# at-cg/PHI

Measured on AMD Instinct MI355X. Metric: read Gbases/s scored (49-hap MHC graph stand-in synMHC-49); reads resident in HBM, parsing and H2D excluded, higher is better.
Workload: dtype u64

## Files before the change

phi_amd/csrc/dp_events.hip:

```cpp
#include <hip/hip_runtime.h>
#include "phi_kernels.h"
#include "dp_dev.h"

#define CHK PHI_DP_CHUNK
#define RING PHI_DP_RING
enum { DP_SEQ = 0, DP_ROW = 1, DP_PATH = 2 };

__global__ void __launch_bounds__(256) phi_event_flags_kernel(const int32_t *__restrict__ walk_vtx, int64_t n_entries,
                                                              const int32_t *__restrict__ cvtx, uint8_t *__restrict__ flags)
{
    for (int64_t e = (int64_t)blockIdx.x * blockDim.x + threadIdx.x; e < n_entries; e += (int64_t)gridDim.x * blockDim.x)
        flags[e] = cvtx[walk_vtx[e]] >= 0;
}

__global__ void phi_event_off_kernel(const phi_ent_t *__restrict__ ev_e, int64_t n_ev, const int64_t *__restrict__ walk_off,
                                     int32_t n_walks, int64_t *__restrict__ ev_off)
{
    const int h = blockIdx.x * blockDim.x + threadIdx.x;
    if (h > n_walks) return;
    const int64_t key = walk_off[h];
    int64_t lo = 0, hi = n_ev;
    while (lo < hi) {
        const int64_t mid = (lo + hi) >> 1;
        if ((int64_t)ev_e[mid] < key) lo = mid + 1; else hi = mid;
    }
    ev_off[h] = lo;
}

void phi_launch_event_flags(hipStream_t st, const int32_t *walk_vtx, int64_t n_entries, const int32_t *cvtx, uint8_t *flags)
{
    if (n_entries <= 0) return;
    int64_t nb = (n_entries + 255) / 256;
    if (nb > 4096) nb = 4096;
    hipLaunchKernelGGL(phi_event_flags_kernel, dim3((unsigned)nb), dim3(256), 0, st, walk_vtx, n_entries, cvtx, flags);
}

void phi_launch_event_off(hipStream_t st, const phi_ent_t *ev_e, int64_t n_ev, const int64_t *walk_off, int32_t n_walks,
                          int64_t *ev_off)
{
    hipLaunchKernelGGL(phi_event_off_kernel, dim3((unsigned)((n_walks + 1 + 63) / 64)), dim3(64), 0, st, ev_e, n_ev,
                       walk_off, n_walks, ev_off);
}

#define EVF_STAGE 3072
__global__ void __launch_bounds__(256) phi_dp_event_fill_kernel(const phi_ent_t *__restrict__ ev_e, int64_t n_ev,
                                                                const int32_t *__restrict__ walk_vtx,
                                                                const int32_t *__restrict__ cvtx,
                                                                const int64_t *__restrict__ walk_off, int32_t n_walks,
                                                                const uint8_t *__restrict__ e_out,
                                                                const int64_t *__restrict__ g_off,
                                                                const uint8_t *__restrict__ g_span,
                                                                const uint8_t *__restrict__ a_weight,
                                                                const phi_ent_t *__restrict__ a_e1,
                                                                const int32_t *__restrict__ wpre, int64_t n_entries,
                                                                uint4 *__restrict__ ev)
{
    __shared__ uint32_t s_e1[EVF_STAGE];
    __shared__ uint8_t s_sw[EVF_STAGE];
    __shared__ int64_t s_rng[2];
    const int64_t n_blocks = (n_ev + 255) / 256;
    for (int64_t blk = blockIdx.x; blk < n_blocks; blk += gridDim.x) {
        const int64_t i = blk * 256 + threadIdx.x;
        const bool in = i < n_ev;
        const int64_t e = ev_e[in ? i : n_ev - 1];
        const int64_t e1st = ((int64_t)__builtin_amdgcn_readfirstlane((int)(e >> 32)) << 32) | (uint32_t)__builtin_amdgcn_readfirstlane((int)(uint32_t)e);
        int lo = phi_walk_of_entry(walk_off, n_walks, e1st);
        if (__ballot(e >= walk_off[lo + 1]) != 0ull) lo = phi_walk_of_entry(walk_off, n_walks, e, lo);
        const int64_t eb = walk_off[lo];
        const int64_t x0 = e - 29 > eb ? e - 29 : eb;
        const int64_t xe = e + 31 < n_entries ? e + 31 : n_entries;
        const int64_t g_lo = g_off[x0], g_e = g_off[e], g_hi = g_off[e + 1], g_fe = g_off[xe];
        if (threadIdx.x == 0) s_rng[0] = g_lo;
        if (i == (n_ev < blk * 256 + 256 ? n_ev : blk * 256 + 256) - 1) s_rng[1] = g_fe;
        __syncthreads();
        const int64_t gb = s_rng[0], ge = s_rng[1];
        const bool staged = ge - gb <= EVF_STAGE;
        if (staged)
            for (int64_t j = threadIdx.x; j < ge - gb; j += 256) {
                s_e1[j] = a_e1[gb + j];
                s_sw[j] = (uint8_t)(g_span[gb + j] | (a_weight[gb + j] ? 0x80 : 0));
            }
        __syncthreads();
        if (in) {
            unsigned long long w[4] = {0, 0, 0, 0};
            int total = 0;
            int32_t sb_extra = 0;
            auto count = [&](int a) {
                if (a > 30) return;
                total++;
                const unsigned long long one = 1ull << (8 * (a & 7));
                if ((a >> 3) == 0) w[0] += one; else if ((a >> 3) == 1) w[1] += one; else if ((a >> 3) == 2) w[2] += one; else w[3] += one;
            };
            const uint32_t e32 = (uint32_t)e;
            if (staged) {
                for (int64_t g = g_lo - gb; g < g_hi - gb; g++) {
                    const uint32_t sw = s_sw[g];
                    if (sw & 0x80) count((int)(e32 - (s_e1[g] - (sw & 0x7F))));
                }
                for (int64_t g = g_e - gb; g < g_fe - gb; g++) {
                    const uint32_t sw = s_sw[g];
                    sb_extra += (sw & 0x80) && (int64_t)s_e1[g] - (int64_t)(sw & 0x7F) < e;
                }
            } else {
                for (int64_t g = g_lo; g < g_hi; g++)
                    if (a_weight[g]) count((int)(e - ((int64_t)a_e1[g] - g_span[g])));
                for (int64_t g = g_e; g < g_fe; g++) sb_extra += a_weight[g] && (int64_t)a_e1[g] - g_span[g] < e;
            }
            const bool ovf = total > 255;
            unsigned long long carry = 0;
#pragma unroll
            for (int q = 0; q < 4; q++) {
                w[q] = w[q] * 0x0101010101010101ull + carry * 0x0101010101010101ull;
                carry = w[q] >> 56;
            }
            w[3] = (w[3] & 0x00FFFFFFFFFFFFFFull) | ((unsigned long long)e_out[e] << 56);
            const int32_t base = wpre[g_off[eb]];
            uint4 A;
            A.x = (uint32_t)cvtx[walk_vtx[e]] | (ovf ? 0x80000000u : 0u);
            A.y = (uint32_t)e;
            A.z = (uint32_t)(wpre[g_hi] - base);
            A.w = (uint32_t)(wpre[g_e] - base + sb_extra);
            ev[i * 3 + 0] = A;
            ev[i * 3 + 1] = make_uint4((uint32_t)w[0], (uint32_t)(w[0] >> 32), (uint32_t)w[1], (uint32_t)(w[1] >> 32));
            ev[i * 3 + 2] = make_uint4((uint32_t)w[2], (uint32_t)(w[2] >> 32), (uint32_t)w[3], (uint32_t)(w[3] >> 32));
        }
        __syncthreads();
    }
}

void phi_launch_dp_event_fill(hipStream_t st, const PhiDpEventArgs &A, const uint8_t *e_out, const int32_t *walk_vtx,
                              const int32_t *cvtx, const phi_ent_t *a_e1, const int32_t *wpre, int64_t n_entries)
{
    if (A.n_ev <= 0) return;
    int64_t nb = (A.n_ev + 255) / 256;
    if (nb > 16384) nb = 16384;
    hipLaunchKernelGGL(phi_dp_event_fill_kernel, dim3((unsigned)nb), dim3(256), 0, st, A.ev_e, A.n_ev, walk_vtx, cvtx,
                       A.walk_off, A.n_walks, e_out, A.g_off, A.g_span, A.a_weight, a_e1, wpre, n_entries,
                       reinterpret_cast<uint4 *>(A.ev));
}

__device__ __forceinline__ unsigned long long ev_key(int32_t val, int lane)
{
    return ((unsigned long long)(uint32_t)(val - NEG) << 8) | (unsigned long long)(255 - lane);
}
__device__ __forceinline__ unsigned long long ev_max_u53(unsigned long long a, unsigned long long b)
{
    double r;
    asm("v_max_f64 %0, %1, %2" : "=v"(r) : "v"(__longlong_as_double((long long)a)), "v"(__longlong_as_double((long long)b)));
    return (unsigned long long)__double_as_longlong(r);
}
#define EV_DPP64(x, ctrl, rm, bc)                                                                                             \
    (((unsigned long long)(uint32_t)__builtin_amdgcn_update_dpp((int)((x) >> 32), (int)((x) >> 32), ctrl, rm, 0xF, bc) << 32) | \
     (uint32_t)__builtin_amdgcn_update_dpp((int)(uint32_t)(x), (int)(uint32_t)(x), ctrl, rm, 0xF, bc))
__device__ __forceinline__ void ev_wave_max2_key(unsigned long long a, unsigned long long b, unsigned long long &ma, unsigned long long &mb)
{
    a = ev_max_u53(a, EV_DPP64(a, 0x121, 0xF, false)); b = ev_max_u53(b, EV_DPP64(b, 0x121, 0xF, false));
    a = ev_max_u53(a, EV_DPP64(a, 0x122, 0xF, false)); b = ev_max_u53(b, EV_DPP64(b, 0x122, 0xF, false));
    a = ev_max_u53(a, EV_DPP64(a, 0x124, 0xF, false)); b = ev_max_u53(b, EV_DPP64(b, 0x124, 0xF, false));
    a = ev_max_u53(a, EV_DPP64(a, 0x128, 0xF, false)); b = ev_max_u53(b, EV_DPP64(b, 0x128, 0xF, false));
    a = ev_max_u53(a, EV_DPP64(a, 0x142, 0xA, false)); b = ev_max_u53(b, EV_DPP64(b, 0x142, 0xA, false));
    a = ev_max_u53(a, EV_DPP64(a, 0x143, 0xC, false)); b = ev_max_u53(b, EV_DPP64(b, 0x143, 0xC, false));
    ma = ((unsigned long long)(uint32_t)__builtin_amdgcn_readlane((int)(a >> 32), 63) << 32) | (uint32_t)__builtin_amdgcn_readlane((int)(uint32_t)a, 63);
    mb = ((unsigned long long)(uint32_t)__builtin_amdgcn_readlane((int)(b >> 32), 63) << 32) | (uint32_t)__builtin_amdgcn_readlane((int)(uint32_t)b, 63);
}

__device__ int32_t ev_count_inside(const PhiDpEventArgs &A, int64_t es, int64_t e)
{
    int32_t n = 0;
    for (int64_t x = es; x <= e; x++)
        for (int64_t g = A.g_off[x]; g < A.g_off[x + 1]; g++)
            if (A.a_weight[g] && x - A.g_span[g] >= es) n++;
    return n;
}

template <int NW, int MODE>
__global__ void __launch_bounds__(NW * 64) phi_dp_events_kernel(PhiDpEventArgs A)
{
    static_assert(NW == 2 || NW == 4, "65..128 or 129..256 walks");
    constexpr int NT = NW * 64;
    constexpr int D = NW == 2 ? 8 : 4;
    constexpr int P = D / 2;
    constexpr int QD = NW == 2 ? 32 : 16;
    constexpr int RNG = NW == 2 ? RING : 512;
    __shared__ int4 s_rec[2][CHK][2];
    __shared__ int4 s_top[RNG];
    __shared__ uint4 s_ev[D][3][NT];
    __shared__ int32_t s_qs[QD][NT], s_qE[QD][NT], s_qK[QD][NT];
    const int32_t q_limit = A.q_limit > 0 && A.q_limit < QD ? A.q_limit : (QD == 32 ? 32 : QD);
    __shared__ unsigned long long s_red[NW];
    __shared__ int32_t s_oidx[NT];

    const int h = threadIdx.x;
    const bool has_walk = h < A.n_walks;
    const int64_t eb = has_walk ? A.walk_off[h] : 0;
    const int64_t ee = has_walk ? A.walk_off[h + 1] : 0;
    const int32_t sb = MODE == DP_PATH ? (int32_t)blockIdx.x : 0;
    const int32_t kbeg = MODE == DP_PATH ? A.blk_lo[sb] : 0, kend = MODE == DP_PATH ? A.blk_lo[sb + 1] : A.n_k;
    const int64_t vb = !has_walk ? 0 : MODE == DP_PATH ? (int64_t)A.blk_ev[(int64_t)sb * A.lane_stride + h] : A.ev_off[h];
    const int64_t ve = has_walk ? A.ev_off[h + 1] : 0;
    int64_t vi = vb;
    int64_t wl = vb;
    const uint4 *evg = reinterpret_cast<const uint4 *>(A.ev);

    uint4 wtmp[P][3];
    int64_t whi = vb;
    auto issue = [&]() {
        whi = min(ve, vi + D);
#pragma unroll
        for (int j = 0; j < P; j++) {
            const int64_t x = (ve > vb) ? min(wl + j, ve - 1) : 0;
            wtmp[j][0] = evg[x * 3 + 0]; wtmp[j][1] = evg[x * 3 + 1]; wtmp[j][2] = evg[x * 3 + 2];
        }
    };
    auto land = [&]() {
#pragma unroll
        for (int j = 0; j < P; j++) {
            const int64_t x = wl + j;
            if (x < whi) {
                const int sl = (int)(x & (D - 1));
                s_ev[sl][0][h] = wtmp[j][0]; s_ev[sl][1][h] = wtmp[j][1]; s_ev[sl][2][h] = wtmp[j][2];
            }
        }
        wl = max(wl, min(whi, wl + P));
    };
    if (A.n_ev > 0) { issue(); land(); issue(); land(); }
    uint4 cA = make_uint4(0xFFFFFFFFu, 0, 0, 0);
    if (vi < ve) cA = s_ev[vi & (D - 1)][0][h];

    int32_t qh = 0, qt = 0;
    int32_t M = NEGK, sL = 0, Emax = NEG;
    if (MODE == DP_PATH) { sL = -1; if (has_walk) M = A.blk_S[(int64_t)sb * A.lane_stride + h]; }

    const int32_t n_steps = kend - kbeg;
    const int n_chunks = (n_steps + CHK - 1) / CHK;
    auto stage = [&](int c) {
        const int b = c & 1;
        const int32_t s0 = kbeg + c * CHK;
        const int32_t ns = min(CHK, kend - s0);
        const int4 *src = reinterpret_cast<const int4 *>(A.k_rec + (int64_t)s0 * 8);
        int4 *dst = &s_rec[b][0][0];
        for (int i = h; i < ns * 2; i += NT) dst[i] = src[i];
    };
    stage(0);
    __syncthreads();

    for (int c = 0; c < n_chunks; c++) {
        const int b = c & 1;
        if (c + 1 < n_chunks) stage(c + 1);
        const int32_t s0 = kbeg + c * CHK;
        const int32_t ns = min(CHK, kend - s0);
        int4 ra = s_rec[b][0][0], rb = s_rec[b][0][1];
        for (int i = 0; i < ns; i++) {
            const int inx = min(i + 1, CHK - 1);
            const int4 na = s_rec[b][inx][0], nb = s_rec[b][inx][1];
            if ((c | i) && (i & (P - 1)) == 0) issue();
            if ((c | i) && (i & (P - 1)) == P / 2) {
                land();
                if (vi < ve) cA = s_ev[vi & (D - 1)][0][h];
            }
            const int32_t k = s0 + i;
            const int32_t flags = ra.x;
            const bool active = (int32_t)(cA.x & 0x7FFFFFFFu) == k;

            int32_t E = NEG, Eh = -1, Esrc = -1;
            if (flags & PHI_DP_NEED_ENTRY) {
                dp_eval_entry<RNG, true>(ra, rb, k, s_top, A.k_in_packed, reinterpret_cast<const int4 *>(A.tops), A.cost, E, Eh, Esrc);
                if (h == 0) { A.ent_src[k] = Esrc; A.ent_h[k] = Eh; }
            }

            int32_t dmax = NEG;
            int32_t oidx = 255;
            if (active) {
                const int64_t e = (int64_t)cA.y;
                const bool ovf = (cA.x >> 31) != 0;
                const int32_t t = (int32_t)(e - eb);
                const int32_t End = (int32_t)cA.z, SB = (int32_t)cA.w;
                const int sl = (int)(vi & (D - 1));
                const uint8_t *gb = reinterpret_cast<const uint8_t *>(&s_ev[sl][1][h]);
                oidx = reinterpret_cast<const uint8_t *>(&s_ev[sl][2][h])[15];
                while (qh != qt && t - s_qs[qh & (QD - 1)][h] >= 31) {
                    const int32_t key = s_qK[qh & (QD - 1)][h];
                    if (key > M) { M = key; sL = s_qs[qh & (QD - 1)][h]; }
                    qh++;
                }
                int32_t newE = NEG;
                if (t == 0) { newE = 0; qh = qt = 0; M = NEGK; Emax = NEG; }
                else if ((flags & PHI_DP_NEED_ENTRY) && Eh >= 0) newE = E;
                if (newE > Emax) {
                    Emax = newE;
                    const int32_t key = newE - SB;
                    while (qh != qt && s_qK[(qt - 1) & (QD - 1)][h] < key) qt--;
                    if (qt - qh >= q_limit) { atomicOr(A.err, PHI_KERR_DP_QUEUE); qt--; }
                    s_qs[qt & (QD - 1)][h] = t; s_qE[qt & (QD - 1)][h] = newE; s_qK[qt & (QD - 1)][h] = key;
                    qt++;
                }
                if ((flags & PHI_DP_NEED_TOPS) || e == ee - 1) {
                    int32_t best = M > NEGK / 2 ? M + End : NEG, bs = sL;
                    for (int32_t j = qh; j != qt; j++) {
                        const int32_t s = s_qs[j & (QD - 1)][h];
                        const int a = t - s;
                        int32_t inside;
                        if (!ovf) inside = a < 16 ? gb[a] : reinterpret_cast<const uint8_t *>(&s_ev[sl][2][h])[a - 16];
                        else inside = ev_count_inside(A, eb + s, e);
                        const int32_t val = s_qE[j & (QD - 1)][h] + inside;
                        if (val > best) { best = val; bs = s; }
                    }
                    if (best > NEG / 2) { dmax = best; A.dmax[e] = best; A.bstart[e] = bs; }
                    else { A.dmax[e] = NEG; A.bstart[e] = 0; }
                }
                vi++;
                cA = make_uint4(0xFFFFFFFFu, 0, 0, 0);
                if (vi < ve) cA = s_ev[vi & (D - 1)][0][h];
            }

            if (flags & PHI_DP_NEED_TOPS) {
                const bool leaving = active && oidx != 255 && dmax > NEG / 2;
                const DpTops t = dp_tops_waves<NW>(leaving, dmax, oidx, s_red, s_oidx);
                if (h == 0) {
                    const int4 q = pack_tops(t);
                    s_top[k & (RNG - 1)] = q;
                    reinterpret_cast<int4 *>(A.tops)[k] = q;
                }
                __syncthreads();
            }
            ra = na; rb = nb;
        }
        __threadfence_block();
        __syncthreads();
    }
    if (MODE == DP_PATH) {
        int32_t best = M > NEGK / 2 ? M : NEGK, bs = sL;
        for (int32_t j = qh; j != qt; j++) {
            const int32_t key = s_qK[j & (QD - 1)][h];
            if (key > best) { best = key; bs = s_qs[j & (QD - 1)][h]; }
        }
        A.blk_keys_out[(int64_t)sb * A.lane_stride + h] = (has_walk && vb < ve) ? best : NEGK;
        A.blk_carry[(int64_t)sb * A.lane_stride + h] = bs;
    }
}


template <int NPW, int MODE, int P, int RINGT, int QD, int CK = CHK>
__global__ void __launch_bounds__(64 * (1 + NPW)) phi_dp_events_pc_kernel(PhiDpEventArgs A)
{
    constexpr int D = 2 * P;
    constexpr int PER_CHUNK = CK / P;
    static_assert(P % NPW == 0 && CK % P == 0, "ring geometry");
    __shared__ int4 s_rec[2 * CK][2];
    __shared__ int4 s_top[RINGT];
    __shared__ int2 s_ent[2 * P];
    __shared__ uint4 s_ev[D][3][64];
    __shared__ int4 s_res[D][64];
    __shared__ int32_t s_qs[QD][64], s_qE[QD][64], s_qK[QD][64];
    __shared__ int32_t s_vi[2][64];

    const int wave = threadIdx.x >> 6, h = threadIdx.x & 63;
    const bool cls = MODE == DP_ROW && A.lane_walk != nullptr;
    const unsigned n_rows = cls ? 65u : (unsigned)(A.n_walks + 1);
    int32_t sb = 0, row_j = -1;
    if (MODE == DP_ROW) { sb = (int32_t)(blockIdx.x / n_rows); row_j = (int32_t)(blockIdx.x % n_rows); }
    if (MODE == DP_PATH) sb = (int32_t)blockIdx.x;
    const bool start_row = MODE == DP_ROW && row_j == (int32_t)n_rows - 1;
    int32_t w = h;
    bool has_walk = h < A.n_walks;
    if (cls) { w = A.lane_walk[(int64_t)sb * 64 + h]; has_walk = w >= 0; if (!has_walk) w = 0; }
    const int32_t k0 = MODE == DP_SEQ ? 0 : A.blk_lo[sb];
    const int32_t k1 = MODE == DP_SEQ ? A.n_k : A.blk_lo[sb + 1];
    const int32_t n_steps = k1 - k0;
    const phi_ent_t eb = has_walk ? (phi_ent_t)A.walk_off[w] : 0;
    const phi_ent_t e_last = has_walk ? (phi_ent_t)(A.walk_off[w + 1] - 1) : 0xFFFFFFFFu;
    const int32_t v0 = has_walk ? (int32_t)A.ev_off[w] : 0;
    const int32_t ve = has_walk ? (int32_t)A.ev_off[w + 1] : 0;
    const int32_t vb = MODE == DP_SEQ ? v0 : (has_walk ? A.blk_ev[(int64_t)sb * A.lane_stride + w] : 0);
    const int n_per = (n_steps + P - 1) / P;
    if (MODE == DP_ROW && !start_row) {
        const int32_t wj = cls ? A.lane_walk[(int64_t)sb * 64 + row_j] : row_j;
        if (wj < 0) return;
        const int32_t jb = A.blk_ev[(int64_t)sb * A.lane_stride + wj];
        if (jb <= (int32_t)A.ev_off[wj] || jb >= (int32_t)A.ev_off[wj + 1]) {
            if (wave == 0) {
                A.row_out[(int64_t)blockIdx.x * 64 + h] = NEGK;
                if (h == 0) { A.rowend_out[blockIdx.x] = NEG; if (A.rownew_out) A.rownew_out[blockIdx.x] = NEGK; if (A.rowdiag_out) A.rowdiag_out[(int64_t)sb * 64 + row_j] = NEGK; }
            }
            return;
        }
    }

    if (wave > 0) {
        const int pw = wave - 1;
        const uint4 *evg = reinterpret_cast<const uint4 *>(A.ev);
        auto stage = [&](int c) {
            const int32_t s0 = k0 + c * CK;
            const int32_t ns = min(CK, k1 - s0);
            const int4 *src = reinterpret_cast<const int4 *>(A.k_rec + (int64_t)s0 * 8);
            int4 *dst = &s_rec[(c & 1) * CK][0];
            for (int i = pw * 64 + h; i < ns * 2; i += 64 * NPW) dst[i] = src[i];
        };
        stage(0);
#pragma unroll
        for (int n = 0; n < D / NPW; n++) {
            const int32_t x = vb + pw + n * NPW;
            if (x < ve) {
                const uint4 a = evg[(int64_t)x * 3 + 0], g0 = evg[(int64_t)x * 3 + 1], g1 = evg[(int64_t)x * 3 + 2];
                s_ev[x & (D - 1)][0][h] = a; s_ev[x & (D - 1)][1][h] = g0; s_ev[x & (D - 1)][2][h] = g1;
            }
        }
        int32_t wl = min(ve, vb + D);
        int32_t vprev = vb;
        __syncthreads();
        for (int p = 0;; p++) {
            const int32_t vi = has_walk ? s_vi[p & 1][h] : 0;
            if (MODE != DP_ROW) {
#pragma unroll
                for (int n = 0; n < P / NPW; n++) {
                    const int32_t x = vprev + pw + n * NPW;
                    if (x < vi) {
                        const int4 r = s_res[x & (D - 1)][h];
                        A.dmax[(phi_ent_t)r.z] = r.x; A.bstart[(phi_ent_t)r.z] = r.y;
                    }
                }
                if (pw == 0 && p > 0 && h < P) {
                    const int32_t r = (p - 1) * P + h;
                    if (r < n_steps) {
                        const int32_t k = k0 + r;
                        reinterpret_cast<int4 *>(A.tops)[k] = s_top[k & (RINGT - 1)];
                        const int2 en = s_ent[r & (2 * P - 1)];
                        A.ent_src[k] = en.x; A.ent_h[k] = en.y;
                    }
                }
            }
            if (p == n_per) break;
            const int32_t hi = min(ve, vi + D);
            uint4 t0[P / NPW], t1[P / NPW], t2[P / NPW];
#pragma unroll
            for (int n = 0; n < P / NPW; n++) {
                const int64_t xc = (ve > v0) ? min(wl + pw + n * NPW, ve - 1) : 0;
                t0[n] = evg[xc * 3 + 0]; t1[n] = evg[xc * 3 + 1]; t2[n] = evg[xc * 3 + 2];
            }
#pragma unroll
            for (int n = 0; n < P / NPW; n++) {
                const int32_t x = wl + pw + n * NPW;
                if (x < hi) { s_ev[x & (D - 1)][0][h] = t0[n]; s_ev[x & (D - 1)][1][h] = t1[n]; s_ev[x & (D - 1)][2][h] = t2[n]; }
            }
            wl = max(wl, min(hi, wl + P));
            if (p % PER_CHUNK == 0 && (p / PER_CHUNK + 1) * CK < n_steps) stage(p / PER_CHUNK + 1);
            vprev = vi;
            __syncthreads();
        }
        return;
    }

    int32_t vi = vb;
    s_vi[0][h] = vi;
    __syncthreads();
    uint4 cA = make_uint4(0xFFFFFFFFu, 0, 0, 0);
    if (vi < ve) cA = s_ev[vi & (D - 1)][0][h];
    int32_t qh = 0, qn = 0, hs = 0, hE = 0, tk = 0;
    int32_t M = NEGK, sL = MODE == DP_SEQ ? 0 : -1, Emax = NEG;
    if (MODE == DP_ROW && h == row_j) M = 0;
    if (MODE == DP_PATH && has_walk) M = A.blk_S[(int64_t)sb * A.lane_stride + h];
    const bool starts_on = MODE != DP_ROW || start_row;
    int32_t endbest = NEG;
    int32_t Kn = NEGK;
    int4 ra = s_rec[0][0], rb = s_rec[0][1];
    int4 lastq = make_int4(NEG, NEG, 0, 0);
    int32_t lastk = -1;

    auto eval_entry = [&](const int4 xa, const int4 xb, int32_t k, int32_t &E, int32_t &Eh, int32_t &Esrc) {
        const uint32_t b0 = (uint32_t)xa.z >> 8;
        if (((xa.x >> 8) & 0xFF) == 1 && b0 < RINGT) {
            const int32_t src = k - (int32_t)b0;
            int32_t val, hh;
            tops_for_edge(src == lastk ? lastq : s_top[src & (RINGT - 1)], xa.z & 0xFF, val, hh);
            E = NEG; Eh = -1; Esrc = -1;
            if (hh >= 0) { E = val - A.cost; Eh = hh; Esrc = src; }
        } else {
            dp_eval_entry<RINGT, MODE != DP_ROW>(xa, xb, k, s_top, A.k_in_packed, reinterpret_cast<const int4 *>(A.tops), A.cost, E, Eh, Esrc);
        }
        if (h == 0) s_ent[(k - k0) & (2 * P - 1)] = make_int2(Esrc, Eh);
    };

    for (int p = 0; p < n_per; p++) {
        const int32_t r_end = min(n_steps, (p + 1) * P);
        if (vi < ve) cA = s_ev[vi & (D - 1)][0][h];
        for (int32_t r = p * P; r < r_end;) {
            const int32_t k = k0 + r;
            const int4 na = s_rec[(r + 1) & (2 * CK - 1)][0], nb = s_rec[(r + 1) & (2 * CK - 1)][1];
            const int4 n2a = s_rec[(r + 2) & (2 * CK - 1)][0], n2b = s_rec[(r + 2) & (2 * CK - 1)][1];
            const bool pair = (ra.x & PHI_DP_PAIR) && r + 1 < r_end;
            const int32_t stepk = (int32_t)(cA.x & 0x7FFFFFFFu);
            const bool second = pair && stepk == k + 1;
            const bool active = stepk == k || second;
            const int32_t flags = second ? na.x : ra.x;

            int32_t E = NEG, Eh = -1, Esrc = -1;
            if (ra.x & PHI_DP_NEED_ENTRY) eval_entry(ra, rb, k, E, Eh, Esrc);
            if (pair && (na.x & PHI_DP_NEED_ENTRY)) {
                int32_t E1, Eh1, Esrc1;
                eval_entry(na, nb, k + 1, E1, Eh1, Esrc1);
                if (second) { E = E1; Eh = Eh1; Esrc = Esrc1; }
            } else if (second) { E = NEG; Eh = -1; }

            int32_t dmax = NEG;
            int32_t oidx = 255;
            if (active) {
                const int sl = (int)(vi & (D - 1));
                const phi_ent_t e = cA.y;
                const bool ovf = (cA.x >> 31) != 0;
                const int32_t t = (int32_t)(e - eb);
                const int32_t End = (int32_t)cA.z, SB = (int32_t)cA.w;
                const uint8_t *gb = reinterpret_cast<const uint8_t *>(&s_ev[sl][1][h]);
                oidx = gb[15 + 1024];
                while (qn > 0 && t - hs >= 31) {
                    const int32_t key = qn == 1 ? tk : s_qK[qh & (QD - 1)][h];
                    if (key > M) { M = key; sL = hs; }
                    qh++; qn--;
                    if (qn > 0) { hs = s_qs[qh & (QD - 1)][h]; hE = s_qE[qh & (QD - 1)][h]; }
                }
                int32_t newE = NEG;
                if (t == 0) { newE = starts_on ? 0 : NEG; qn = 0; M = NEGK; Emax = NEG; }
                else if ((flags & PHI_DP_NEED_ENTRY) && Eh >= 0) newE = E;
                if (newE > Emax) {
                    Emax = newE;
                    const int32_t key = newE - SB;
                    while (qn > 0 && tk < key) {
                        qn--;
                        if (qn > 0) tk = s_qK[(qh + qn - 1) & (QD - 1)][h];
                    }
                    if (QD < 32 && qn == QD) { atomicOr(A.err, PHI_KERR_DP_QUEUE); qn--; }
                    const int slq = (qh + qn) & (QD - 1);
                    s_qs[slq][h] = t; s_qE[slq][h] = newE; s_qK[slq][h] = key;
                    if (qn == 0) { hs = t; hE = newE; }
                    tk = key;
                    qn++;
                    if (MODE == DP_ROW && key > Kn) Kn = key;
                }
                int32_t bs = 0;
                if ((flags & PHI_DP_NEED_TOPS) || e == e_last) {
                    int32_t best = M > NEGK / 2 ? M + End : NEG;
                    bs = sL;
                    for (int32_t j = 0; j < qn; j++) {
                        const int32_t s = j == 0 ? hs : s_qs[(qh + j) & (QD - 1)][h];
                        const int32_t Es = j == 0 ? hE : s_qE[(qh + j) & (QD - 1)][h];
                        const int a = t - s;
                        const int32_t inside = !ovf ? (int32_t)gb[(a & 15) + (a >> 4) * 1024] : ev_count_inside(A, (int64_t)eb + s, e);
                        const int32_t val = Es + inside;
                        if (val > best) { best = val; bs = s; }
                    }
                    if (best > NEG / 2) dmax = best; else bs = 0;
                    if (MODE == DP_ROW && e == e_last) endbest = max(endbest, dmax);
                }
                s_res[sl][h] = make_int4(dmax, bs, (int32_t)e, 0);
                vi++;
                cA = make_uint4(0xFFFFFFFFu, 0, 0, 0);
                if (vi < ve) cA = s_ev[vi & (D - 1)][0][h];
            }

            if (!pair && (ra.x & PHI_DP_NEED_TOPS)) {
                const bool leaving = active && oidx != 255 && dmax > NEG / 2;
                DpTops t;
                if (__ballot(leaving && oidx > 1) == 0ull) {
                    const bool on0 = leaving && oidx == 0, on1 = leaving && oidx == 1;
                    unsigned long long K0, K1;
                    ev_wave_max2_key(on0 ? ev_key(dmax, h) : 0ull, on1 ? ev_key(dmax, h) : 0ull, K0, K1);
                    const bool first0 = K0 >= K1;
                    const unsigned long long Kf = first0 ? K0 : K1, Ks = first0 ? K1 : K0;
                    t.t1v = Kf ? (int32_t)(uint32_t)(Kf >> 8) + NEG : NEG;
                    t.t1h = Kf ? 255 - (int32_t)(Kf & 255) : -1;
                    t.t1n = Kf ? (first0 ? 0 : 1) : -1;
                    t.t2v = Ks ? (int32_t)(uint32_t)(Ks >> 8) + NEG : NEG;
                    t.t2h = Ks ? 255 - (int32_t)(Ks & 255) : -1;
                } else {
                    t = dp_tops_wave(leaving, dmax, oidx);
                }
                lastq = pack_tops(t);
                lastk = k;
                if (h == 0) s_top[k & (RINGT - 1)] = lastq;
            }
            if (pair) { ra = n2a; rb = n2b; r += 2; }
            else { ra = na; rb = nb; r += 1; }
        }
        s_vi[(p + 1) & 1][h] = vi;
        __syncthreads();
    }
    if (MODE != DP_SEQ) {
        int32_t best = M > NEGK / 2 ? M : NEGK, bs = sL;
        for (int32_t j = 0; j < qn; j++) {
            const int32_t key = s_qK[(qh + j) & (QD - 1)][h];
            if (key > best) { best = key; bs = s_qs[(qh + j) & (QD - 1)][h]; }
        }
        if (MODE == DP_ROW) {
            const bool on_diag = A.rowdiag_out && h == row_j;
            if (on_diag) A.rowdiag_out[(int64_t)sb * 64 + h] = has_walk ? best : NEGK;
            A.row_out[(int64_t)blockIdx.x * 64 + h] = has_walk && !on_diag ? best : NEGK;
            const int32_t eb_all = wave_max_i32(endbest);
            if (h == 0) A.rowend_out[blockIdx.x] = eb_all;
            if (A.rownew_out && h == row_j) A.rownew_out[blockIdx.x] = Kn;
            if (A.rownew_out && start_row && h == 0) A.rownew_out[blockIdx.x] = NEGK;
        } else {
            A.blk_keys_out[(int64_t)sb * A.lane_stride + h] = (has_walk && vb < ve) ? best : NEGK;
            A.blk_carry[(int64_t)sb * A.lane_stride + h] = bs;
        }
    }
}

void phi_launch_dp_block_paths_wide(hipStream_t st, const PhiDpEventArgs &A)
{
    if (A.n_walks <= 128) hipLaunchKernelGGL((phi_dp_events_kernel<2, DP_PATH>), dim3((unsigned)A.n_blk), dim3(128), 0, st, A);
    else hipLaunchKernelGGL((phi_dp_events_kernel<4, DP_PATH>), dim3((unsigned)A.n_blk), dim3(256), 0, st, A);
}

void phi_launch_dp_events(hipStream_t st, const PhiDpEventArgs &A)
{
    if (A.n_walks <= 64) hipLaunchKernelGGL((phi_dp_events_pc_kernel<2, DP_SEQ, 8, RING, 32>), dim3(1), dim3(64 * 3), 0, st, A);
    else if (A.n_walks <= 128) hipLaunchKernelGGL((phi_dp_events_kernel<2, DP_SEQ>), dim3(1), dim3(128), 0, st, A);
    else hipLaunchKernelGGL((phi_dp_events_kernel<4, DP_SEQ>), dim3(1), dim3(256), 0, st, A);
}

void phi_launch_dp_block_rows(hipStream_t st, const PhiDpEventArgs &A)
{
    const unsigned grid = (unsigned)A.n_blk * (A.lane_walk ? 65u : (unsigned)(A.n_walks + 1));
    if (A.blk_ring <= 256 && A.blk_max_len > 0 && A.blk_max_len <= 64 && !getenv("PHI_DP_ROWS_LARGE"))
        hipLaunchKernelGGL((phi_dp_events_pc_kernel<2, DP_ROW, 2, 64, 8, 32>), dim3(grid), dim3(64 * 3), 0, st, A);
    else if (A.blk_ring <= 256) hipLaunchKernelGGL((phi_dp_events_pc_kernel<2, DP_ROW, 2, 256, 8>), dim3(grid), dim3(64 * 3), 0, st, A);
    else if (A.blk_ring <= 1024) hipLaunchKernelGGL((phi_dp_events_pc_kernel<2, DP_ROW, 4, 1024, 16>), dim3(grid), dim3(64 * 3), 0, st, A);
    else hipLaunchKernelGGL((phi_dp_events_pc_kernel<2, DP_ROW, 4, 2048, 16>), dim3(grid), dim3(64 * 3), 0, st, A);
}
void phi_launch_dp_block_paths(hipStream_t st, const PhiDpEventArgs &A)
{
    if (A.blk_ring <= 256) hipLaunchKernelGGL((phi_dp_events_pc_kernel<2, DP_PATH, 4, 256, 8>), dim3((unsigned)A.n_blk), dim3(64 * 3), 0, st, A);
    else if (A.blk_ring <= 1024) hipLaunchKernelGGL((phi_dp_events_pc_kernel<2, DP_PATH, 4, 1024, 16>), dim3((unsigned)A.n_blk), dim3(64 * 3), 0, st, A);
    else hipLaunchKernelGGL((phi_dp_events_pc_kernel<2, DP_PATH, 4, 2048, 16>), dim3((unsigned)A.n_blk), dim3(64 * 3), 0, st, A);
}

__global__ void phi_warm_dp_events_kernel() {}
void phi_warm_dp_events(hipStream_t st) { hipLaunchKernelGGL(phi_warm_dp_events_kernel, dim3(1), dim3(64), 0, st); }
```

Measured before the change: 473.7.

## Shrink DP_ROW pc kernel to two waves and drop unused LDS writes

For DP_ROW mode the kernel no longer writes per-step entry records (s_ent) or per-event results (s_res) to shared memory, since row mode uses only endbest. The two small-ring DP_ROW launches change template parameters (first and third arguments from 2 to 1, plus an explicit 64 for the 256 ring) and drop from three waves to two per block. This is meant to cut LDS footprint and block size so more row blocks fit per CU. Less pipelining depth per block is the cost, and correctness depends on DP_ROW never reading s_res/s_ent. A profiling A/B script is also added.

```diff
diff --git a/phi_amd/csrc/dp_events.hip b/phi_amd/csrc/dp_events.hip
--- a/phi_amd/csrc/dp_events.hip
+++ b/phi_amd/csrc/dp_events.hip
@@ -477,7 +477,7 @@
         } else {
             dp_eval_entry<RINGT, MODE != DP_ROW>(xa, xb, k, s_top, A.k_in_packed, reinterpret_cast<const int4 *>(A.tops), A.cost, E, Eh, Esrc);
         }
-        if (h == 0) s_ent[(k - k0) & (2 * P - 1)] = make_int2(Esrc, Eh);
+        if (MODE != DP_ROW && h == 0) s_ent[(k - k0) & (2 * P - 1)] = make_int2(Esrc, Eh);
     };
 
     for (int p = 0; p < n_per; p++) {
@@ -550,7 +550,7 @@
                     if (best > NEG / 2) dmax = best; else bs = 0;
                     if (MODE == DP_ROW && e == e_last) endbest = max(endbest, dmax);
                 }
-                s_res[sl][h] = make_int4(dmax, bs, (int32_t)e, 0);
+                if (MODE != DP_ROW) s_res[sl][h] = make_int4(dmax, bs, (int32_t)e, 0);
                 vi++;
                 cA = make_uint4(0xFFFFFFFFu, 0, 0, 0);
                 if (vi < ve) cA = s_ev[vi & (D - 1)][0][h];
@@ -621,8 +621,8 @@
 {
     const unsigned grid = (unsigned)A.n_blk * (A.lane_walk ? 65u : (unsigned)(A.n_walks + 1));
     if (A.blk_ring <= 256 && A.blk_max_len > 0 && A.blk_max_len <= 64 && !getenv("PHI_DP_ROWS_LARGE"))
-        hipLaunchKernelGGL((phi_dp_events_pc_kernel<2, DP_ROW, 2, 64, 8, 32>), dim3(grid), dim3(64 * 3), 0, st, A);
-    else if (A.blk_ring <= 256) hipLaunchKernelGGL((phi_dp_events_pc_kernel<2, DP_ROW, 2, 256, 8>), dim3(grid), dim3(64 * 3), 0, st, A);
+        hipLaunchKernelGGL((phi_dp_events_pc_kernel<1, DP_ROW, 1, 64, 8, 32>), dim3(grid), dim3(64 * 2), 0, st, A);
+    else if (A.blk_ring <= 256) hipLaunchKernelGGL((phi_dp_events_pc_kernel<1, DP_ROW, 1, 256, 8, 64>), dim3(grid), dim3(64 * 2), 0, st, A);
     else if (A.blk_ring <= 1024) hipLaunchKernelGGL((phi_dp_events_pc_kernel<2, DP_ROW, 4, 1024, 16>), dim3(grid), dim3(64 * 3), 0, st, A);
     else hipLaunchKernelGGL((phi_dp_events_pc_kernel<2, DP_ROW, 4, 2048, 16>), dim3(grid), dim3(64 * 3), 0, st, A);
 }
diff --git a/profiles/dp_rows_rate.py b/profiles/dp_rows_rate.py
--- /dev/null
+++ b/profiles/dp_rows_rate.py
@@ -0,0 +1,194 @@
+import argparse
+import csv
+import ctypes
+import glob
+import hashlib
+import json
+import os
+import re
+import subprocess
+import sys
+import tempfile
+import time
+
+ROOT = os.path.dirname(os.path.dirname(os.path.abspath(__file__)))
+THIS_LIB = os.path.join(ROOT, "phi_amd", "libphi_amd.so")
+BENCH = [sys.executable, os.path.join(ROOT, "bench.py")]
+T0 = time.time()
+
+
+def occupancy_child(lib):
+    names = [l.split()[-1] for l in subprocess.check_output(["nm", "-D", "--defined-only", lib], text=True).splitlines()
+             if re.search(r" V _Z\d+phi_dp_events_pc_kernelILi\d+ELi1E", l)]
+    out = {}
+    try:
+        L = ctypes.CDLL(lib)
+        hip = None
+        for so in ("libamdhip64.so", "libamdhip64.so.7", "libamdhip64.so.6", os.path.join(os.environ.get("ROCM_PATH", "/opt/rocm"), "lib", "libamdhip64.so")):
+            try:
+                hip = ctypes.CDLL(so)
+                break
+            except OSError:
+                pass
+        for name in sorted(names):
+            handle = ctypes.c_void_p(ctypes.addressof(ctypes.c_char.in_dll(L, name)))
+            n = ctypes.c_int(-1)
+            err = hip.hipOccupancyMaxActiveBlocksPerMultiprocessor(ctypes.byref(n), handle, ctypes.c_int(192), ctypes.c_size_t(0))
+            out[name] = n.value if err == 0 else f"hip error {err}"
+    except Exception as e:
+        out["error"] = repr(e)
+    print(json.dumps(out), flush=True)
+
+
+class Stop(Exception):
+    pass
+
+
+def run(cmd, limit_s, env=None, budget=None):
+    if budget is not None and time.time() - T0 + limit_s > budget:
+        raise Stop(f"budget: {limit_s} s for `{' '.join(cmd[-6:])}` no longer fit")
+    t0 = time.time()
+    r = subprocess.run(["timeout", "-k", "10", str(limit_s)] + cmd, capture_output=True, text=True, env=env, cwd=ROOT)
+    dt = time.time() - t0
+    print(f"[dp_rows_rate] {dt:6.1f} s rc {r.returncode}: {' '.join(cmd[-8:])}", flush=True)
+    if r.returncode != 0:
+        raise Stop(f"exit {r.returncode} after {dt:.0f} s: {' '.join(cmd)}: {r.stderr[-600:]}")
+    return r, dt
+
+
+def env_for(lib):
+    e = dict(os.environ)
+    e.pop("PHI_AMD_LIB", None)
+    if lib != THIS_LIB:
+        e["PHI_AMD_LIB"] = lib
+    return e
+
+
+def traced(lib, bench_args, limit_s, budget):
+    with tempfile.TemporaryDirectory(prefix="dp_rows_") as d:
+        _, dt = run(["rocprofv3", "--kernel-trace", "--stats", "-f", "csv", "-d", d, "-o", "t", "--"] + BENCH + bench_args, limit_s, env_for(lib), budget)
+        rec = {"seconds": dt, "kernels": {}}
+        for f in glob.glob(os.path.join(d, "**", "*kernel_stats.csv"), recursive=True):
+            for row in csv.DictReader(open(f)):
+                m = re.search(r"phi_dp_events_pc_kernel<([\d, ]+)>", row["Name"])
+                if m or "phi_dp_event_fill_kernel" in row["Name"]:
+                    key = "pc<" + m.group(1).replace(" ", "") + ">" if m else "event_fill"
+                    rec["kernels"][key] = {"calls": int(row["Calls"]), "total_ns": int(row["TotalDurationNs"]), "avg_ns": float(row["AverageNs"])}
+        for f in glob.glob(os.path.join(d, "**", "*kernel_trace.csv"), recursive=True):
+            for row in csv.DictReader(open(f)):
+                m = re.search(r"phi_dp_events_pc_kernel<([\d, ]+)>", row.get("Kernel_Name", ""))
+                if m:
+                    key = "pc<" + m.group(1).replace(" ", "") + ">"
+                    rec["kernels"].setdefault(key, {}).update({c.lower(): row[c] for c in ("LDS_Block_Size", "Workgroup_Size", "Grid_Size", "VGPR_Count", "Scratch_Size") if c in row})
+        return rec
+
+
+def bench_line(lib, bench_args, limit_s, budget, timing=True):
+    e = env_for(lib)
+    if timing:
+        e["PHI_TIMING"] = "1"
+    r, dt = run(BENCH + bench_args, limit_s, e, budget)
+    line = json.loads([l for l in r.stdout.splitlines() if l.startswith("{")][-1])
+    laps = [float(x) for x in re.findall(r"\[phi timing\] solve:\s+DP run \+ backtrack\s+([\d.]+) ms", r.stderr)]
+    rec = {"seconds": dt, "value": line.get("value"), "index_build_s": line.get("index_build_s"), "solve_s": line.get("solve_s"), "gpu_path_s": line.get("gpu_path_s"),
+           "ms_per_step": line.get("ms_per_step"), "result": line.get("result"), "parity_checked": line.get("parity_checked"),
+           "dp_run_backtrack_ms": {"n": len(laps), "median": sorted(laps)[len(laps) // 2] if laps else None, "min": min(laps) if laps else None, "max": max(laps) if laps else None}}
+    return rec
+
+
+def digest_dir(d):
+    return {os.path.basename(f): hashlib.md5(open(f, "rb").read()).hexdigest() for f in sorted(glob.glob(os.path.join(d, "*")))}
+
+
+def summarise(vals_parent, vals_this):
+    if not vals_parent or not vals_this:
+        return None
+    med = lambda v: sorted(v)[len(v) // 2]
+    spread = max(max(vals_parent) - min(vals_parent), max(vals_this) - min(vals_this))
+    diff = med(vals_parent) - med(vals_this)
+    return {"median_parent": med(vals_parent), "median_this": med(vals_this), "larger_spread": spread, "difference_of_medians": diff,
+            "no_overlap": max(vals_this) < min(vals_parent), "more_than_twice_the_spread": diff > 2 * spread}
+
+
+def main():
+    ap = argparse.ArgumentParser()
+    ap.add_argument("--occupancy", metavar="LIB", help="(child) print the occupancy of LIB's DP_ROW instances")
+    ap.add_argument("--parent-lib", help="libphi_amd.so of the parent commit")
+    ap.add_argument("--extra-lib", action="append", default=[], metavar="NAME=PATH", help="one more build in the alternation (an experiment)")
+    ap.add_argument("--rounds", type=int, default=3)
+    ap.add_argument("--budget-s", type=float, default=1000.0, help="start no step that would end later than this")
+    ap.add_argument("--solve-args", default="--gpus 1 --steps 200 --warmup 20 --no-cpu-baseline")
+    ap.add_argument("--c5", action="store_true")
+    ap.add_argument("--parity", action="store_true", help="one run of this build with the CPU baseline (parity_checked)")
+    ap.add_argument("--out", default=os.path.join(ROOT, "profiles", "dp_rows_lds_ab.json"))
+    args = ap.parse_args()
+    if args.occupancy:
+        return occupancy_child(args.occupancy)
+    libs = {"parent": os.path.abspath(args.parent_lib), "this": THIS_LIB}
+    libs.update({x.split("=", 1)[0]: os.path.abspath(x.split("=", 1)[1]) for x in args.extra_lib})
+    out = {"what": __doc__.split("\n\n")[0].replace("\n", " "), "occupancy": {}, "kernel": {n: [] for n in libs}, "solve": {n: [] for n in libs}}
+
+    def save():
+        os.makedirs(os.path.dirname(os.path.abspath(args.out)), exist_ok=True)
+        with open(args.out, "w") as f:
+            json.dump(out, f, indent=1)
+
+    trace_args = "--steps 5 --warmup 1 --no-cpu-baseline --no-extra-legs".split()
+    try:
+        for name, lib in libs.items():
+            r, _ = run([sys.executable, os.path.abspath(__file__), "--occupancy", lib], 60, env_for(lib), args.budget_s)
+            out["occupancy"][name] = json.loads(r.stdout.splitlines()[-1])
+            save()
+        t_trace, t_solve = 240, 400
+        for rnd in range(args.rounds):
+            order = list(libs.items())[::-1] if rnd % 2 else list(libs.items())
+            for name, lib in order:
+                rec = traced(lib, trace_args, t_trace, args.budget_s)
+                out["kernel"][name].append(rec)
+                t_trace = min(t_trace, int(rec["seconds"] * 2 + 30))
+                save()
+            for name, lib in order:
+                rec = bench_line(lib, args.solve_args.split(), t_solve, args.budget_s)
+                out["solve"][name].append(rec)
+                t_solve = min(t_solve, int(rec["seconds"] * 2 + 30))
+                save()
+        with tempfile.TemporaryDirectory(prefix="dp_rows_out_") as d:
+            sums = {}
+            for name, lib in libs.items():
+                run(BENCH + trace_args + ["--dump-outputs", os.path.join(d, name)], t_trace, env_for(lib), args.budget_s)
+                sums[name] = digest_dir(os.path.join(d, name))
+            out["dump_outputs"] = {"md5": sums, "identical": sums["parent"] == sums["this"] and len(sums["this"]) > 0}
+            save()
+        if args.parity:
+            out["parity_run"] = bench_line(libs["this"], "--gpus 1 --steps 20 --warmup 5 --no-extra-legs".split(), 300, args.budget_s, timing=False)
+            save()
+        if args.c5:
+            c5_args = "--config C5 --steps 2 --warmup 1 --no-cpu-baseline --no-extra-legs --job-repeats 0".split()
+            out["c5_kernel"] = {}
+            for name, lib in libs.items():
+                out["c5_kernel"][name] = traced(lib, c5_args, 420, args.budget_s)
+                save()
+    except Stop as e:
+        out["stopped"] = str(e)
+        print("[dp_rows_rate] stopped:", e, flush=True)
+
+    def rows_ns(recs):
+        return [k["avg_ns"] for rec in recs for key, k in rec["kernels"].items() if re.match(r"pc<\d,1,\d,256,", key) and "avg_ns" in k]
+    laps = {n: [r["dp_run_backtrack_ms"]["median"] for r in out["solve"][n] if r["dp_run_backtrack_ms"]["median"] is not None] for n in libs}
+
+    def criterion(a, b):
+        return {"rows_ring_256_ns": summarise(rows_ns(out["kernel"][a]), rows_ns(out["kernel"][b])),
+                "dp_run_backtrack_ms": summarise(laps[a], laps[b]),
+                "solve_s": summarise([r["solve_s"] for r in out["solve"][a]], [r["solve_s"] for r in out["solve"][b]]),
+                "gpu_path_s": summarise([r["gpu_path_s"] for r in out["solve"][a]], [r["gpu_path_s"] for r in out["solve"][b]])}
+    out["criterion"] = criterion("parent", "this")
+    out["criterion"]["value_gbases_per_s"] = {n: [r["value"] for r in out["solve"][n]] for n in libs}
+    for n in list(libs)[2:]:
+        out["criterion_this_to_" + n] = criterion("this", n)
+    save()
+    print(json.dumps({k: v for k, v in out.items() if k.startswith("criterion")}, indent=1))
+    return 1 if "stopped" in out else 0
+
+
+if __name__ == "__main__":
+    sys.exit(main())
```

After: 475.8, median of 5. About the same (+0.4%).
